# zhouxian/act3d-chained-diffuser

Measured on AMD Instinct MI355X. Metric: train samples/sec (Act3D keypose fwd+bwd+AdamW step), higher is better.
Workload: dtype fp16 / bf16 MFMA on two-part operands (x = hi + lo; fp32 accumulate) in attention; fp32-accurate linears (f32 MFMA; bf16x3 MFMA from 4096 rows); bf16 frozen backbone + FPN; 1 GPU; Act3D keypose training step, 18-PerAct-task shapes: 4 cameras 256x256, 3 ghost-point levels, 1000 ghost points (333/level), E=60, frozen synthetic CLIP-RN50-shaped backbone + trainable FPN included in the step; per_gpu_batch_keyframes=64, global_batch=64, parallelism=dp1, hipgraph=True, backbone_prefetch=True

## Files before the change

act3d-chained-diffuser_amd/csrc/conv3x3.hip:

```cpp
#include "a3d_common.h"
#include "../../include/act3d_hip.h"

namespace a3d {

constexpr int C3_TH = 8, C3_TW = 32;
constexpr int C3_HW = C3_TW + 2, C3_HP = (C3_TH + 2) * C3_HW;
constexpr int C3_XL = (C3_HP * 4 + 255) / 256;

__device__ __forceinline__ int c3_woff(int row, int seg) { return row * 32 + ((seg ^ (((row >> 1) & 1) | (((row >> 4) & 1) << 1))) << 3); }
__device__ __forceinline__ int c3_xoff(int hp, int hx, int seg) { return hp * 32 + ((seg ^ ((hx >> 1) & 3)) << 3); }

typedef float c3_f32x2 __attribute__((ext_vector_type(2)));
typedef short c3_s16x2 __attribute__((ext_vector_type(2)));
typedef unsigned int c3_u32x4 __attribute__((ext_vector_type(4)));

struct C3Cursor {
  int img, ty, tx;
  __device__ __forceinline__ void advance(int dimg, int dty, int dtx, int tiles_y, int tiles_x) {
    tx += dtx;
    if (tx >= tiles_x) { tx -= tiles_x; ++ty; }
    ty += dty;
    if (ty >= tiles_y) { ty -= tiles_y; ++img; }
    img += dimg;
  }
};

constexpr int c3_lds_bytes(int halves, int nt) { return halves * 9 * 16 * nt * 64 + 2 * C3_HP * 64 + 2 * 32 * halves * 4; }

template <int HALVES, int NT, int D, bool LIST = false>
__global__ __launch_bounds__(256, (2 * c3_lds_bytes(HALVES, NT) <= 160 * 1024 ? 2 : 1)) void conv3x3_stream_kernel(
    const unsigned short* __restrict__ x, const unsigned short* __restrict__ w, const float* __restrict__ in_scale,
    const float* __restrict__ in_shift, int in_relu, unsigned short* __restrict__ y, float* __restrict__ partial, int nimg, int H,
    int W, int ctot, const int* __restrict__ tlist = nullptr) {
  constexpr int CIN = 32 * HALVES, COUT = 16 * NT;
  const int co0 = blockIdx.y * COUT;
  static_assert(D % HALVES == 0, "the half of a step must be a compile-time function of its slot");
  extern __shared__ __attribute__((aligned(16))) unsigned short smem_c3[];
  unsigned short* Ws = smem_c3;
  unsigned short* Xs = Ws + HALVES * 9 * COUT * 32;
  float* scS = reinterpret_cast<float*>(Xs + 2 * C3_HP * 32);
  const int t = threadIdx.x, lane = t & 63, wave = t >> 6;
  const int li = lane & 15, g = lane >> 4;
  const int nwg = gridDim.x;
  const int lb = (nwg & 7) == 0 ? (int)(blockIdx.x & 7) * (nwg >> 3) + (int)(blockIdx.x >> 3) : (int)blockIdx.x;
  const int tiles_x = W / C3_TW, tiles_y = H / C3_TH, tpi = tiles_x * tiles_y;
  const int ntiles = LIST ? __builtin_amdgcn_readfirstlane(tlist[-2]) : nimg * tpi;
  for (int i = t; i < HALVES * 9 * COUT * 4; i += 256) {
    const int seg = i & 3, r = i >> 2, co = r % COUT, tap = (r / COUT) % 9, h = r / (COUT * 9);
    *reinterpret_cast<uint4*>(&Ws[c3_woff((h * 9 + tap) * COUT + co, seg)]) =
        *reinterpret_cast<const uint4*>(w + ((size_t)(co0 + co) * 9 + tap) * CIN + h * 32 + seg * 8);
  }
  for (int i = t; i < CIN; i += 256) { scS[i] = in_scale ? in_scale[i] : 1.f; scS[CIN + i] = in_scale ? in_shift[i] : 0.f; }
  const int seg_t = t & 3;
  int hy[C3_XL], hx[C3_XL];
#pragma unroll
  for (int i = 0; i < C3_XL; ++i) {
    const int hp = (t + i * 256) >> 2;
    hy[i] = hp / C3_HW;
    hx[i] = hp - hy[i] * C3_HW;
  }
  c3_f32x2 ssum[NT][2], ssq[NT][2];
#pragma unroll
  for (int a = 0; a < NT; ++a)
#pragma unroll
    for (int r = 0; r < 2; ++r) { ssum[a][r] = c3_f32x2{0.f, 0.f}; ssq[a][r] = c3_f32x2{0.f, 0.f}; }
  const int my_tiles = lb < ntiles ? (ntiles - lb + nwg - 1) / nwg : 0;
  const int total = my_tiles * HALVES;
  const int dimg = nwg / tpi, dty = (nwg - dimg * tpi) / tiles_x, dtx = nwg - dimg * tpi - dty * tiles_x;
  C3Cursor cl;
  auto from_list = [&](int ordinal) {
    const int e = __builtin_amdgcn_readfirstlane(tlist[lb + ordinal * nwg]);
    return C3Cursor{e >> 16, (e >> 8) & 255, e & 255};
  };
  if (LIST) {
    cl = my_tiles > 0 ? from_list(0) : C3Cursor{0, 0, 0};
  } else {
    cl.img = lb / tpi;
    cl.ty = (lb - cl.img * tpi) / tiles_x;
    cl.tx = lb - cl.img * tpi - cl.ty * tiles_x;
  }
  C3Cursor cc = cl;
  int lk = 0, lhalf = 0;
  int ck = 0;
  auto load_next = [&](uint4 (&r)[C3_XL]) {
    const int y0 = cl.ty * C3_TH, x0 = cl.tx * C3_TW;
    const char* base = reinterpret_cast<const char*>(x + (size_t)cl.img * H * W * CIN + lhalf * 32);
#pragma unroll
    for (int i = 0; i < C3_XL; ++i) {
      const int iy = min(max(y0 - 1 + hy[i], 0), H - 1), ix = min(max(x0 - 1 + hx[i], 0), W - 1);
      const unsigned int off = (unsigned int)((iy * W + ix) * CIN + seg_t * 8) * 2u;
      r[i] = *reinterpret_cast<const uint4*>(base + off);
    }
    if (++lhalf == HALVES) {
      lhalf = 0;
      if (lk + 1 < my_tiles) {
        ++lk;
        if (LIST) cl = from_list(lk); else cl.advance(dimg, dty, dtx, tiles_y, tiles_x);
      }
    }
  };
  const c3_s16x2 relu_lo = in_relu ? c3_s16x2{0, 0} : c3_s16x2{(short)-32768, (short)-32768};
  auto stage = [&](int buf, int half, const uint4 (&r)[C3_XL]) {
    const int y0 = cc.ty * C3_TH, x0 = cc.tx * C3_TW;
    const int k0 = half * 32 + seg_t * 8;
    c3_f32x2 sc[4], sh[4];
#pragma unroll
    for (int j = 0; j < 4; ++j) {
      sc[j] = c3_f32x2{scS[k0 + 2 * j], scS[k0 + 2 * j + 1]};
      sh[j] = c3_f32x2{scS[CIN + k0 + 2 * j], scS[CIN + k0 + 2 * j + 1]};
    }
#pragma unroll
    for (int i = 0; i < C3_XL; ++i) {
      const int hp = (t + i * 256) >> 2;
      const int iy = y0 - 1 + hy[i], ix = x0 - 1 + hx[i];
      const bool inside = (unsigned)iy < (unsigned)H && (unsigned)ix < (unsigned)W;
      unsigned int u[4] = {r[i].x, r[i].y, r[i].z, r[i].w};
#pragma unroll
      for (int j = 0; j < 4; ++j) {
        c3_f32x2 v = {__uint_as_float(u[j] << 16), __uint_as_float(u[j] & 0xFFFF0000u)};
        v = v * sc[j] + sh[j];
        const c3_s16x2 pk = __builtin_elementwise_max(__builtin_bit_cast(c3_s16x2, pk_bf16(v.x, v.y)), relu_lo);
        u[j] = inside ? __builtin_bit_cast(unsigned int, pk) : 0u;
      }
      if (hp < C3_HP) *reinterpret_cast<c3_u32x4*>(&Xs[buf * C3_HP * 32 + c3_xoff(hp, hx[i], seg_t)]) = c3_u32x4{u[0], u[1], u[2], u[3]};
    }
  };
  int xo[4][3], woff[NT];
#pragma unroll
  for (int tm = 0; tm < 4; ++tm)
#pragma unroll
    for (int kw = 0; kw < 3; ++kw) {
      const int col = (tm & 1) * 16 + li + kw;
      xo[tm][kw] = c3_xoff((2 * wave + (tm >> 1)) * C3_HW + col, col, g);
    }
#pragma unroll
  for (int tn = 0; tn < NT; ++tn) woff[tn] = c3_woff((li >> 2) * (4 * NT) + tn * 4 + (li & 3), g);
  if (total > 0) {
    uint4 xr[D][C3_XL];
#pragma unroll
    for (int j = 0; j < D; ++j) load_next(xr[j]);
    f32x4 acc[NT][4];
#pragma unroll
    for (int a = 0; a < NT; ++a)
#pragma unroll
      for (int b = 0; b < 4; ++b) acc[a][b] = f32x4{0.f, 0.f, 0.f, 0.f};
    __syncthreads();
    for (int s0 = 0; s0 < total; s0 += D) {
#pragma unroll
      for (int j = 0; j < D; ++j) {
        const int s = s0 + j;
        if (s >= total) break;
        const int half = j % HALVES, buf = s & 1;
        stage(buf, half, xr[j]);
        load_next(xr[j]);
        __syncthreads();
        const unsigned short* Xb = Xs + buf * C3_HP * 32;
        const unsigned short* Wb = Ws + half * 9 * COUT * 32;
        auto taps_of_row = [&](int kh) {
#pragma unroll
          for (int kw = 0; kw < 3; ++kw) {
            s16x8 xa[4], wb[NT];
#pragma unroll
            for (int tm = 0; tm < 4; ++tm) xa[tm] = *reinterpret_cast<const s16x8*>(&Xb[xo[tm][kw] + kh * (C3_HW * 32)]);
#pragma unroll
            for (int tn = 0; tn < NT; ++tn) wb[tn] = *reinterpret_cast<const s16x8*>(&Wb[(kh * 3 + kw) * COUT * 32 + woff[tn]]);
#pragma unroll
            for (int tn = 0; tn < NT; ++tn)
#pragma unroll
              for (int tm = 0; tm < 4; ++tm) acc[tn][tm] = mfma_bf16_16x16x32(wb[tn], xa[tm], acc[tn][tm]);
          }
        };
#pragma unroll
        for (int kh = 0; kh < 3; ++kh) taps_of_row(kh);
        if (half == HALVES - 1) {
          const int y0 = cc.ty * C3_TH, x0 = cc.tx * C3_TW;
#pragma unroll
          for (int tm = 0; tm < 4; ++tm) {
            const int oy = y0 + 2 * wave + (tm >> 1), ox = x0 + (tm & 1) * 16 + li;
            unsigned int pk[2 * NT];
#pragma unroll
            for (int tn = 0; tn < NT; ++tn) {
#pragma unroll
              for (int r2 = 0; r2 < 2; ++r2) {
                const unsigned int u = pk_bf16(acc[tn][tm][2 * r2], acc[tn][tm][2 * r2 + 1]);
                const c3_f32x2 v = {__uint_as_float(u << 16), __uint_as_float(u & 0xFFFF0000u)};
                ssum[tn][r2] += v;
                ssq[tn][r2] += v * v;
                pk[2 * tn + r2] = u;
              }
              acc[tn][tm] = f32x4{0.f, 0.f, 0.f, 0.f};
            }
            char* ybase = reinterpret_cast<char*>(y + (size_t)cc.img * H * W * ctot + co0);
            c3_u32x4* dst = reinterpret_cast<c3_u32x4*>(ybase + (unsigned int)((oy * W + ox) * ctot + g * (4 * NT)) * 2u);
#pragma unroll
            for (int q = 0; q < NT / 2; ++q) dst[q] = c3_u32x4{pk[4 * q], pk[4 * q + 1], pk[4 * q + 2], pk[4 * q + 3]};
          }
          if (LIST) { if (++ck < my_tiles) cc = from_list(ck); } else cc.advance(dimg, dty, dtx, tiles_y, tiles_x);
        }
      }
    }
  }
  if (LIST) {
    const int nzero = __builtin_amdgcn_readfirstlane(tlist[-1]);
    const int last = nimg * tpi - 1;
    for (int k = lb; k < nzero; k += nwg) {
      const int e = __builtin_amdgcn_readfirstlane(tlist[last - k]);
      const int img = e >> 16, oy = ((e >> 8) & 255) * C3_TH + (t >> 5), ox = (e & 255) * C3_TW + (t & 31);
      char* ybase = reinterpret_cast<char*>(y + (size_t)img * H * W * ctot + co0);
      c3_u32x4* dst = reinterpret_cast<c3_u32x4*>(ybase + (unsigned int)((oy * W + ox) * ctot) * 2u);
#pragma unroll
      for (int q = 0; q < COUT / 8; ++q) dst[q] = c3_u32x4{0u, 0u, 0u, 0u};
    }
  }
  if (!partial) return;
  __syncthreads();
  float* redS = reinterpret_cast<float*>(Xs);
  float* redQ = redS + 4 * COUT;
#pragma unroll
  for (int tn = 0; tn < NT; ++tn)
#pragma unroll
    for (int r = 0; r < 4; ++r) {
      float sv = ssum[tn][r >> 1][r & 1], q = ssq[tn][r >> 1][r & 1];
#pragma unroll
      for (int o = 1; o < 16; o <<= 1) { sv += __shfl_xor(sv, o, 64); q += __shfl_xor(q, o, 64); }
      if (li == 0) { redS[wave * COUT + g * (4 * NT) + tn * 4 + r] = sv; redQ[wave * COUT + g * (4 * NT) + tn * 4 + r] = q; }
    }
  __syncthreads();
  if (t < COUT) {
    float sv = 0.f, q = 0.f;
#pragma unroll
    for (int j = 0; j < 4; ++j) { sv += redS[j * COUT + t]; q += redQ[j * COUT + t]; }
    float* p = partial + (size_t)blockIdx.x * 2 * ctot + co0;
    p[t] = sv;
    p[ctot + t] = q;
  }
}

__global__ __launch_bounds__(256) void c3_mark_tiles_kernel(const long long* __restrict__ idx, long long ntok, int k, int ncam, int H,
                                                          int W, unsigned char* __restrict__ mask) {
  const long long i = (long long)blockIdx.x * 256 + threadIdx.x;
  if (i >= ntok) return;
  const long long p = idx[i];
  const int b = (int)(i / k);
  const int cam = (int)(p / ((long long)H * W));
  const int rem = (int)(p - (long long)cam * H * W);
  const int h = rem / W, w0 = rem - h * W;
  const int tiles_x = W / C3_TW, tiles_y = H / C3_TH;
  const int img = b * ncam + cam;
  const int ty0 = max(h - 1, 0) / C3_TH, ty1 = min(h + 1, H - 1) / C3_TH, tx0 = max(w0 - 1, 0) / C3_TW, tx1 = min(w0 + 1, W - 1) / C3_TW;
  for (int ty = ty0; ty <= ty1; ++ty)
    for (int tx = tx0; tx <= tx1; ++tx) mask[((size_t)img * tiles_y + ty) * tiles_x + tx] = 1;
}

__global__ __launch_bounds__(1024) void c3_compact_tiles_kernel(const unsigned char* __restrict__ mask, int ntiles, int tiles_x,
                                                              int tiles_y, int* __restrict__ tlist) {
  __shared__ int wsum[16];
  __shared__ int carry;
  const int t = threadIdx.x, lane = t & 63, wave = t >> 6;
  const int tpi = tiles_x * tiles_y;
  if (t == 0) carry = 0;
  __syncthreads();
  for (int base = 0; base < ntiles; base += 1024) {
    const int id = base + t;
    const int on = (id < ntiles && mask[id]) ? 1 : 0;
    const unsigned long long bal = __ballot(on);
    const int before = __popcll(bal & ((1ull << lane) - 1ull));
    if (lane == 0) wsum[wave] = __popcll(bal);
    __syncthreads();
    int off = carry;
    for (int w2 = 0; w2 < wave; ++w2) off += wsum[w2];
    if (id < ntiles) {
      const int img = id / tpi, r = id - img * tpi, ty = r / tiles_x, tx = r - ty * tiles_x;
      const int e = (img << 16) | (ty << 8) | tx;
      const int pos_on = off + before;
      if (on) tlist[pos_on] = e; else tlist[ntiles - 1 - (id - pos_on)] = e;
    }
    __syncthreads();
    if (t == 0) { int tot = 0; for (int w2 = 0; w2 < 16; ++w2) tot += wsum[w2]; carry += tot; }
    __syncthreads();
  }
  if (t == 0) { tlist[-2] = carry; tlist[-1] = ntiles - carry; }
}

}

using namespace a3d;

static int c3_cblock(int Cin, int Cout) {
  static const bool split = !(getenv("A3D_C3_SPLIT") && atoi(getenv("A3D_C3_SPLIT")) == 0);
  return (Cin == 64 && Cout == 64 && split) ? 32 : Cout;
}
static size_t c3_lds(int Cin, int Cout) { return (size_t)c3_lds_bytes(Cin / 32, c3_cblock(Cin, Cout) / 16); }
static bool c3_serves(int Cin, int Cout, int H, int W) {
  const bool ch = (Cin == 32 && (Cout == 32 || Cout == 64)) || (Cin == 64 && Cout == 64);
  return ch && H > 0 && W > 0 && (H % C3_TH) == 0 && (W % C3_TW) == 0;
}
static int c3_slabs(size_t nimg, int H, int W, int Cin, int Cout) {
  const size_t ntiles = nimg * (size_t)(H / C3_TH) * (size_t)(W / C3_TW);
  const int per_cu = 2 * c3_lds(Cin, Cout) <= 160 * 1024 ? 2 : 1;
  const int yblocks = Cout / c3_cblock(Cin, Cout);
  return (int)std::min<size_t>(ntiles, (size_t)std::max(8, 256 * per_cu / yblocks));
}

extern "C" int a3d_conv3x3_serves(int Cin, int Cout, int H, int W) { return c3_serves(Cin, Cout, H, W) ? 1 : 0; }

extern "C" int a3d_conv3x3_nslab(size_t nimg, int H, int W, int Cin, int Cout) {
  if (nimg == 0 || !c3_serves(Cin, Cout, H, W)) return 0;
  return c3_slabs(nimg, H, W, Cin, Cout);
}

extern "C" int a3d_conv3x3_bn_fwd(const void* x, const void* w, const float* in_scale, const float* in_shift, int in_relu, void* y,
                                  float* partial, size_t nimg, int H, int W, int Cin, int Cout, void* stream) {
  if (!x || !w || !y || nimg == 0 || nimg * (size_t)(H > 0 ? H : 1) * (size_t)(W > 0 ? W : 1) / 256 >= (size_t)(1 << 30) || (size_t)(H > 0 ? H : 1) * (size_t)(W > 0 ? W : 1) * 128 >= ((size_t)1 << 31) || !c3_serves(Cin, Cout, H, W) || (in_scale && !in_shift) ||
      ((((uintptr_t)x | (uintptr_t)w | (uintptr_t)y) & 15) != 0)) {
    set_error("a3d_conv3x3_bn_fwd: bad argument (images=%zu H=%d W=%d Cin=%d Cout=%d; served: 32 -> 32, 32 -> 64, 64 -> 64 channels, "
              "H a multiple of 8, W a multiple of 32 -- a3d_conv3x3_serves; 16-byte aligned operands)", nimg, H, W, Cin, Cout);
    return A3D_ERR_ARG;
  }
  hipStream_t s = (hipStream_t)stream;
  const unsigned short* xs = (const unsigned short*)x;
  const unsigned short* ws = (const unsigned short*)w;
  unsigned short* ys = (unsigned short*)y;
  const int slabs = c3_slabs(nimg, H, W, Cin, Cout);
  const size_t lds = c3_lds(Cin, Cout);
#define A3D_C3S(HV, NTV, DV)                                                                                                        \
  do {                                                                                                                           \
    static bool once = false;                                                                                                    \
    if (!once) { (void)hipFuncSetAttribute((const void*)conv3x3_stream_kernel<HV, NTV, DV>, hipFuncAttributeMaxDynamicSharedMemorySize, 128 * 1024); once = true; } \
    hipLaunchKernelGGL((conv3x3_stream_kernel<HV, NTV, DV>), dim3(slabs, Cout / c3_cblock(Cin, Cout)), dim3(256), lds, s, xs, ws, in_scale, in_shift, in_relu, ys, partial, (int)nimg, H, W, Cout); \
  } while (0)
  if (Cin == 32 && Cout == 32) A3D_C3S(1, 2, 3);
  else if (Cin == 32 && Cout == 64) A3D_C3S(1, 4, 2);
  else if (c3_cblock(Cin, Cout) == 32) A3D_C3S(2, 2, 2);
  else A3D_C3S(2, 4, 2);
#undef A3D_C3S
  return check_launch("a3d_conv3x3_bn_fwd");
}

extern "C" size_t a3d_conv3x3_tile_count(size_t nimg, int H, int W) {
  return (H > 0 && W > 0 && (H % C3_TH) == 0 && (W % C3_TW) == 0) ? nimg * (size_t)(H / C3_TH) * (size_t)(W / C3_TW) : 0;
}
extern "C" size_t a3d_conv3x3_dgrad_tiles_ws_ints(size_t nimg, int H, int W) { return a3d_conv3x3_tile_count(nimg, H, W) + 4; }

extern "C" int a3d_conv3x3_mark_tiles(const long long* idx, int B, int k, int ncam, int H, int W, unsigned char* mask, void* stream) {
  if (!idx || !mask || B <= 0 || k <= 0 || ncam <= 0 || a3d_conv3x3_tile_count(1, H, W) == 0 || H / C3_TH > 255 || W / C3_TW > 255) {
    set_error("a3d_conv3x3_mark_tiles: bad argument (B=%d k=%d ncam=%d H=%d W=%d; H a multiple of 8, W of 32)", B, k, ncam, H, W);
    return A3D_ERR_ARG;
  }
  const long long ntok = (long long)B * k;
  hipLaunchKernelGGL(c3_mark_tiles_kernel, dim3((unsigned)((ntok + 255) / 256)), dim3(256), 0, (hipStream_t)stream, idx, ntok, k, ncam, H, W, mask);
  return check_launch("a3d_conv3x3_mark_tiles");
}

extern "C" int a3d_conv3x3_dgrad_tiles(const void* dy, const void* wt, const unsigned char* mask, int* ws, void* dx, size_t nimg, int H,
                                       int W, void* stream) {
  if (!dy || !wt || !mask || !ws || !dx || nimg == 0 || nimg >= 32768 || !c3_serves(64, 64, H, W) || H / C3_TH > 255 || W / C3_TW > 255 ||
      (size_t)H * (size_t)W * 128 >= ((size_t)1 << 31) || ((((uintptr_t)dy | (uintptr_t)wt | (uintptr_t)dx) & 15) != 0)) {
    set_error("a3d_conv3x3_dgrad_tiles: bad argument (images=%zu H=%d W=%d; 64 channels, H a multiple of 8, W of 32, < 32768 images)", nimg, H, W);
    return A3D_ERR_ARG;
  }
  hipStream_t s = (hipStream_t)stream;
  const int ntiles = (int)a3d_conv3x3_tile_count(nimg, H, W);
  int* tlist = ws + 2;
  hipLaunchKernelGGL(c3_compact_tiles_kernel, dim3(1), dim3(1024), 0, s, mask, ntiles, W / C3_TW, H / C3_TH, tlist);
  int rc = check_launch("a3d_conv3x3_dgrad_tiles(compact)");
  if (rc) return rc;
  const int slabs = c3_slabs(nimg, H, W, 64, 64);
  const size_t lds = c3_lds(64, 64);
  const int cb = c3_cblock(64, 64);
  static bool once = false;
  if (cb == 32) {
    if (!once) { (void)hipFuncSetAttribute((const void*)conv3x3_stream_kernel<2, 2, 2, true>, hipFuncAttributeMaxDynamicSharedMemorySize, 128 * 1024); once = true; }
    hipLaunchKernelGGL((conv3x3_stream_kernel<2, 2, 2, true>), dim3(slabs, 2), dim3(256), lds, s, (const unsigned short*)dy, (const unsigned short*)wt,
                       (const float*)nullptr, (const float*)nullptr, 0, (unsigned short*)dx, (float*)nullptr, (int)nimg, H, W, 64, (const int*)tlist);
  } else {
    if (!once) { (void)hipFuncSetAttribute((const void*)conv3x3_stream_kernel<2, 4, 2, true>, hipFuncAttributeMaxDynamicSharedMemorySize, 128 * 1024); once = true; }
    hipLaunchKernelGGL((conv3x3_stream_kernel<2, 4, 2, true>), dim3(slabs, 1), dim3(256), lds, s, (const unsigned short*)dy, (const unsigned short*)wt,
                       (const float*)nullptr, (const float*)nullptr, 0, (unsigned short*)dx, (float*)nullptr, (int)nimg, H, W, 64, (const int*)tlist);
  }
  return check_launch("a3d_conv3x3_dgrad_tiles");
}
```

include/act3d_hip.h:

```cpp
#ifndef ACT3D_HIP_H
#define ACT3D_HIP_H
#include <stddef.h>
#include <stdint.h>
#ifdef __cplusplus
extern "C" {
#endif

int a3d_version(void);
const char* a3d_last_error_string(void);

int a3d_linear_fwd(const float* X, int ldx, const float* W, int ldw, const float* bias, float* Y, int ldy,
                   const float* mask, int ldm, int M, int N, int K, int act, int w_transposed, void* stream);
int a3d_linear_wgrad(const float* dY, int lddy, const float* X, int ldx, float* dW, int lddw, float* db, int M,
                     int N, int K, void* stream);
size_t a3d_linear_wgrad_ws_bytes(int M, int N, int K, int has_bias);
int a3d_linear_wgrad_ws(const float* dY, int lddy, const float* X, int ldx, float* dW, int lddw, float* db, int M,
                        int N, int K, float* ws, size_t ws_bytes, void* stream);
int a3d_add_layernorm_fwd(const float* A, const float* R, const float* gamma, const float* beta, float* Y,
                          float* mean, float* rstd, int M, int E, float eps, void* stream);
int a3d_add_layernorm_bwd(const float* A, const float* R, const float* gamma, const float* mean, const float* rstd,
                          const float* dY, float* dS, float* dgamma, float* dbeta, int M, int E, void* stream);

int a3d_linear_wgrad_partials(const float* dY, int lddy, const float* X, int ldx, int has_bias, int M, int N, int K,
                              float* ws, size_t ws_bytes, int* nsplit_out, void* stream);
int a3d_add_layernorm_bwd_partials_count(int M, int E);
int a3d_add_layernorm_bwd_partials(const float* A, const float* R, const float* gamma, const float* mean, const float* rstd,
                                   const float* dY, float* dS, float* partials, int M, int E, void* stream);
int a3d_colsum_rows_partials(const float* src, int B, int S, int k, int ld, int C, float* ws, void* stream);
typedef struct {
  const float* partial;
  float* dst;
  float* bias;
  int nsplit, slab_stride, count, row_len, dst_stride, group_len;
} A3dGradReduceRec;
int a3d_grad_reduce_table_plan(const A3dGradReduceRec* host_table, int nrec, int* nwg_out);
int a3d_grad_reduce_table_upload(A3dGradReduceRec* dev_table, const A3dGradReduceRec* host_table, int nrec, void* stream);
int a3d_grad_reduce_table(const A3dGradReduceRec* dev_table, int nrec, int nwg, void* stream);

int a3d_rope_split_qk(const float* Y, int ldy, const float* xyz, const float* freq, float scale, void* dst, int B,
                      int N, int Npad, int E, int H, void* stream);
int a3d_split_vt(const float* Y, int ldy, void* dst, int B, int N, int Npad, int E, int H, void* stream);
int a3d_rope_split(const float* Y, int ldy, const float* xyz, const float* freq, float scale, void* rows_out,
                   int rows_width, void* planes_out, int B, int N, int Npad, int E, int H, void* stream);
int a3d_proj_rope_split(const float* X, int ldx, const float* W, int ldw, const float* bias, int K, const float* xyz0,
                        float scale0, void* rows0, int rows0_width, void* planes0, const float* xyz1, float scale1,
                        void* rows1, int rows1_width, void* planes1, const float* freq, int B, int N, int Npad, int E,
                        int H, void* stream);
int a3d_rope_merge_bwd(const float* dR, int nsplit, const float* xyz, const float* freq, float scale, float* dY,
                       int ldy, int B, int N, int Npad, int E, int H, void* stream);

int a3d_attn_fwd(const void* Qs, const void* Ks, const void* Vt, const unsigned char* kmask, float* O, float* LSE,
                 float* ws, int B, int H, int Lq, int Lqp, int S, int Sp, int nsplit, void* stream);
size_t a3d_attn_fwd_ws_floats(int B, int H, int Lqp, int nsplit);
int a3d_attn_bwd_bf16(const void* Qs, const void* Qt, const void* Ks, const void* Kt, const void* Vs,
                      const unsigned char* kmask, const float* O, const float* dO, const float* LSE, void* dOs,
                      void* dOt, float* D, float* dQp, float* dK, float* dV, int B, int H, int Lq, int Lqp, int S,
                      int Sp, int nsplit, void* stream);

int a3d_dropout(const float* x, float* y, size_t n, const unsigned long long* drop_state, unsigned int site, float p,
                void* stream);
int a3d_linear_fwd_drop(const float* X, int ldx, const float* W, int ldw, const float* bias, float* Y, int ldy,
                        const float* mask, int ldm, int M, int N, int K, int act, int w_transposed,
                        const unsigned long long* drop_state, unsigned int site, float p, void* stream);
int a3d_add_layernorm_bwd_drop(const float* A, const float* R, const float* gamma, const float* mean, const float* rstd,
                               const float* dY, float* dS, float* dS_drop, float* dgamma, float* dbeta, int M, int E,
                               const unsigned long long* drop_state, unsigned int site, float p, void* stream);
int a3d_dropout_mask(unsigned char* out, size_t n, const unsigned long long* drop_state, unsigned int c2, unsigned int c1,
                     unsigned int site, float p, void* stream);
int a3d_rope_split16(const float* Y, int ldy, const float* xyz, const float* freq, float scale, void* rows_out,
                     void* planes_out, int plane_parts, int B, int N, int Npad, int E, int H, void* stream);
int a3d_proj_rope_split16(const float* X, int ldx, const float* W, int ldw, const float* bias, int K, const float* xyz0,
                          float scale0, void* rows0, void* planes0, int parts0, const float* xyz1, float scale1, void* rows1,
                          void* planes1, int parts1, const float* freq, int B, int N, int Npad, int E, int H, void* stream);
int a3d_ctx_kv_proj16_splits(int B, int Npad);
int a3d_ctx_kv_proj16(const float* X, int ldx, const float* xyz, const float* W0, const float* bias0, void* Krows0, void* Vrows0,
                      const float* W1, const float* bias1, void* Krows1, void* Vrows1, int ldw, const float* freq, int nl, int B,
                      int N, int Npad, int E, int H, int nsplit, void* stream);
int a3d_attn16_fwd(const void* Qr, const void* Kr, const void* Vp, const unsigned char* kmask, float* O, float* LSE2,
                   float* ws, int B, int H, int Lq, int Lqp, int S, int Sp, int nsplit,
                   const unsigned long long* drop_state, unsigned int drop_site, float drop_p, void* stream);
int a3d_attn16_fwd_rows(const void* Qr, const void* Kr, const void* Vr, const unsigned char* kmask, float* O, float* LSE2,
                        float* ws, int B, int H, int Lq, int Lqp, int S, int Sp, int nsplit,
                        const unsigned long long* drop_state, unsigned int drop_site, float drop_p, int nograd, void* stream);
size_t a3d_attn16_bwd_pack_bytes(int B, int H, int Lqp);
int a3d_attn16_bwd(const void* Qr, const void* Qp, const void* Kr, const void* Kp, const void* Vr,
                   const unsigned char* kmask, const float* O, const float* dO, const float* LSE2, void* dOr, void* pack,
                   float* D, int* rexp, float* dQp, float* dK, float* dV, int B, int H, int Lq, int Lqp, int S, int Sp,
                   int nsplit, const unsigned long long* drop_state, unsigned int drop_site, float drop_p, void* stream);

size_t a3d_attn8_operand_bytes(int B, int H, int Sp);
int a3d_attn8_fwd(const void* Qr, const void* Kr, const void* Vp, void* ops8, const unsigned char* kmask, float* O,
                  float* LSE2, float* ws, int B, int H, int Lq, int Lqp, int S, int Sp, int nsplit, void* stream);

int a3d_attn_fwd_dropout(const void* Qs, const void* Ks, const void* Vt, const unsigned char* kmask, float* O, float* LSE,
                         float* ws, int B, int H, int Lq, int Lqp, int S, int Sp, int nsplit,
                         const unsigned long long* drop_state, unsigned int site, float p, void* stream);
int a3d_attn_bwd_bf16_dropout(const void* Qs, const void* Qt, const void* Ks, const void* Kt, const void* Vs,
                              const unsigned char* kmask, const float* O, const float* dO, const float* LSE, void* dOs,
                              void* dOt, float* D, float* dQp, float* dK, float* dV, int B, int H, int Lq, int Lqp, int S,
                              int Sp, int nsplit, const unsigned long long* drop_state, unsigned int site, float p,
                              void* stream);

size_t a3d_sq_fwd_ws_floats(int B, int H, int E, int nsplit);
int a3d_sq_attn_fwd(const float* X, const float* xyz, const float* Wk, int ldw, const float* bk, const float* Wv, int ldwv,
                    const float* bv, const float* qrot, const float* freq, float* ws, float* xbar, float* lse, float* o, int B,
                    int S, int E, int H, int nsplit, void* stream);
size_t a3d_sq_bwd_ws_floats(int B, int H, int E, int nsplit);
int a3d_sq_attn_bwd(const float* X, const float* xyz, const float* Wk, int ldw, const float* bk, const float* Wv, int ldwv,
                    const float* qrot, const float* freq, const float* xbar, const float* lse, const float* dO, float* ws,
                    float* dX, float* dqp, float* dWk, int lddwk, float* dbk, float* dWv, int lddwv, float* dbv, int B, int S,
                    int E, int H, int nsplit, void* stream);
int a3d_sq_attn_bwd_acc(const float* X, const float* xyz, const float* Wk, int ldw, const float* bk, const float* Wv, int ldwv,
                        const float* qrot, const float* freq, const float* xbar, const float* lse, const float* dO, float* ws,
                        float* dX, float* dqp, float* dWk, int lddwk, float* dbk, float* dWv, int lddwv, float* dbv, int B, int S,
                        int E, int H, int nsplit, int accumulate_dX, void* stream);
int a3d_sq_wgrad_reduce(const float* partial, int nsplit, float* dW, int lddw, float* db, int E, void* stream);

int a3d_pcd_downsample(const float* pcd, float* out_xyz, int B, int C, int Hin, int Win, int factor, void* stream);
size_t a3d_knn_topk_ws_bytes(int B, int N);
int a3d_knn_topk(const float* pos, const float* xyz, void* ws, long long* idx_out, float* dist_out, int B, int N,
                 int k, void* stream);
int a3d_traj_nn_topk(const float* traj_xyz, int L, const float* xyz, void* ws, long long* idx_out, float* dist_out, int B,
                     int N, int k, void* stream);
int a3d_build_context(const float* feat, const long long* idx, const float* extra, float* ctx, int B, int Npts,
                      int k, int X, int W, void* stream);
int a3d_build_context_bwd(const float* dctx, const long long* idx, float* dfeat, float* dextra, int B, int Npts,
                          int k, int X, int W, int accumulate, void* stream);

int a3d_build_context_bf16(const void* feat, int ldf, const long long* idx, const float* extra, const float* bias, float* ctx,
                           int B, int Npts, int k, int X, int W, void* stream);
int a3d_build_context_bwd_bf16(const float* dctx, const long long* idx, void* dfeat, int ldf, float* dextra, int B,
                               int Npts, int k, int X, int W, int accumulate, void* stream);
size_t a3d_conv3x3_wgrad_tokens_ws_floats(void);
int a3d_conv3x3_wgrad_tokens(const void* X, const long long* idx, const float* G, int g_rows, int E, float* ws, float* dW,
                             int accumulate, int B, int k, int ncam, int H, int W, void* stream);
size_t a3d_conv3x3_tile_count(size_t images, int H, int W);
size_t a3d_conv3x3_dgrad_tiles_ws_ints(size_t images, int H, int W);
int a3d_conv3x3_mark_tiles(const long long* idx, int B, int k, int ncam, int H, int W, unsigned char* mask, void* stream);
int a3d_conv3x3_dgrad_tiles(const void* dy, const void* wt, const unsigned char* mask, int* ws, void* dx, size_t images, int H, int W,
                            void* stream);
size_t a3d_colsum_rows_ws_floats(int B, int k, int C);
int a3d_colsum_rows(const float* src, int B, int S, int k, int ld, int C, float* out, int nout, float* ws, void* stream);

int a3d_mask_logits_fwd(const float* q, const float* F, float* out, int B, int Ng, int E, void* stream);
int a3d_mask_logits_bwd(const float* q, const float* F, const float* dlog, float* dF, float* dq, int B, int Ng,
                        int E, int accumulate_dF, void* stream);
int a3d_argmax_gather(const float* logits, const float* ghost, long long* top_idx, float* pos, int B, int Ng,
                      void* stream);
int a3d_soft_ce_loss(const float* ghost, const float* gt, const float* logits, float* loss_b, float* loss,
                     float* dlogits, int B, int Ng, float spread, float label_smoothing, float coeff, void* stream);
int a3d_elem_loss(const float* pred, const float* target, int n, int kind, float coeff, float* loss, float* grad,
                  void* stream);
int a3d_scale_by_scalar(const float* x, const float* scalar, float* y, size_t n, void* stream);
int a3d_quat_sigmoid_fwd(const float* pred, float* rot, float* grip, int B, void* stream);
int a3d_quat_sigmoid_bwd(const float* pred, const float* drot, const float* dgrip, float* dpred, int B, void* stream);
int a3d_ortho6d_sigmoid_fwd(const float* pred, float* rot, float* grip, int B, void* stream);
int a3d_ortho6d_sigmoid_bwd(const float* pred, const float* drot, const float* dgrip, float* dpred, int B, void* stream);
int a3d_select_row_fwd(const float* x, const long long* idx, float* y, int B, int N, int W, void* stream);
int a3d_select_row_bwd(const float* dy, const long long* idx, float* dx, int B, int N, int W, void* stream);
int a3d_sample_ghost_points(const unsigned long long* state, const float* bounds, const float* anchor, float radius,
                            float* out, int B, int Ng, int level, int max_attempts, void* stream);
int a3d_rng_advance(unsigned long long* state, unsigned long long n, void* stream);
void a3d_philox4x32_10_host(const uint32_t* ctr, const uint32_t* key, uint32_t* out);
void a3d_sincos_host(const float* x, float* sn, float* cs, size_t n);
int a3d_adamw_step(float* p, const float* g, float* m, float* v, float* step, const long long* seg_off, float* seg_state,
                   int nseg, size_t n, size_t n_nodecay, float lr, float beta1, float beta2, float eps, float wd_nodecay,
                   float wd_decay, float grad_scale, void* stream);
int a3d_adamw_ema_step(float* p, const float* g, float* m, float* v, float* ema, float* step, const long long* seg_off,
                       float* seg_state, float* ema_state, int nseg, size_t n, size_t n_nodecay, float lr, float beta1, float beta2,
                       float eps, float wd_nodecay, float wd_decay, float grad_scale, float ema_decay, float ema_warmup,
                       void* stream);
#define A3D_ADAMW_CLIP_WS_DOUBLES 256
int a3d_adamw_clip_step(float* p, const float* g, float* m, float* v, float* ema, float* step, const long long* seg_off,
                        float* seg_state, float* ema_state, float* clip_state, double* clip_ws, int nseg, size_t n, size_t n_nodecay,
                        float lr, float beta1, float beta2, float eps, float wd_nodecay, float wd_decay, float grad_scale,
                        float ema_decay, float ema_warmup, float max_norm, void* stream);
#define A3D_LR_CONSTANT 0
#define A3D_LR_LINEAR 1
#define A3D_LR_COSINE 2
int a3d_adamw_sched_step(float* p, const float* g, float* m, float* v, float* ema, float* step, const long long* seg_off,
                         float* seg_state, float* ema_state, float* clip_state, double* clip_ws, float* lr_state, int nseg, size_t n,
                         size_t n_nodecay, int decay_kind, double warmup_steps, double total_steps, double min_ratio, float beta1,
                         float beta2, float eps, float wd_nodecay, float wd_decay, float grad_scale, float ema_decay, float ema_warmup,
                         float max_norm, void* stream);
int a3d_swap_f32(float* a, float* b, size_t n, void* stream);

typedef struct {
  const float *wv, *bv;
  const float *wo, *bo;
  const float *g1, *b1;
  const float *w1, *c1, *w2, *c2;
  const float *g2, *b2;
} a3d_qs_params;
typedef struct {
  float *dwv, *dbv, *dwo, *dbo, *dg1, *db1, *dw1, *dc1, *dw2, *dc2, *dg2, *db2;
} a3d_qs_grads;
int a3d_qs_pre_fwd(const float* x, const float* wq, const float* bq, const float* xyz, const float* freq, float scale, float* qrot,
                   int B, int E, int H, void* stream);
int a3d_qs_pre_bwd(const float* dqp, int nsplit, const float* xyz, const float* freq, float scale, const float* x, const float* wq,
                   float* dwq, float* dbq, float* dx, int B, int E, int H, void* stream);
size_t a3d_qs_save_floats(int B, int E);
int a3d_qs_post_fwd(const float* xbar, const float* resid, const a3d_qs_params* p, float* save, float* y, int B, int E, int H,
                    void* stream);
int a3d_qs_post_bwd(const float* dy, const float* resid, const float* xbar, const float* save, const a3d_qs_params* p,
                    const a3d_qs_grads* gr, float* dxbar, float* cD, float* dresid, int B, int E, int H, void* stream);

int a3d_ddpm_add_noise(const float* x0, const float* noise, const long long* t, const float* acp_pos,
                       const float* acp_rot, float* out, int B, int L, int D, int npos, void* stream);
int a3d_ddpm_step(const float* model_out, const float* sample, const float* noise, const float* cond_data,
                  const unsigned char* cond_mask, const float* coef_pos, const float* coef_rot, float* out, int rows,
                  int D, int npos, int t, void* stream);
int a3d_ddpm_step_sched(const float* model_out, const float* sample, const float* noise, const float* cond_data,
                        const unsigned char* cond_mask, const float* coef_pos, const float* coef_rot, float* out, int rows,
                        int D, int npos, int row, int terminal, void* stream);
int a3d_ddpm_step_hist(const float* model_out, const float* sample, const float* noise, const float* cond_data,
                       const unsigned char* cond_mask, const float* coef_pos, const float* coef_rot, float* out, int rows,
                       int D, int npos, int row, int terminal, float* hist, const float* kappa_pos, const float* kappa_rot,
                       void* stream);
int a3d_adaln_fwd(const float* x, const float* mod, float* y, int B, int L, int E, void* stream);
int a3d_adaln_bwd(const float* x, const float* mod, const float* dy, float* dx, float* dmod, int B, int L, int E,
                  void* stream);
int a3d_sinusoidal_emb(const float* x, float* out, int n, int E, void* stream);
int a3d_silu_fwd(const float* x, float* y, size_t n, void* stream);
int a3d_silu_bwd(const float* x, const float* dy, float* dx, size_t n, void* stream);
int a3d_add_rows(const float* x, const float* r, float* y, int B, int L, int E, void* stream);
int a3d_add_rows_bwd(const float* dy, float* dr, int B, int L, int E, void* stream);
int a3d_traj_update(const float* traj, const float* upd, float* out, int rows, int D, int npos, void* stream);

int a3d_pose_to_signal(const float* pose, const float* bounds, float* out, int n, int extra, void* stream);
int a3d_signal_to_pose(const float* signal, const float* bounds, float* out, int n, int extra, void* stream);
int a3d_traj_condition(const float* curr, int ldc, const float* goal, int ldg, const float* bounds, const unsigned char* tmask,
                       const float* init_noise, float* cg, float* gg, float* cond_data, unsigned char* cond_mask,
                       unsigned char* kmask, float* traj, int B, int G, int L, int Dp, int use_goal, void* stream);
#define A3D_TRAJ_PINS_MAX 32
int a3d_traj_pins(const float* poses, int ldp, const int* index, const unsigned char* channels, const float* bounds,
                  const unsigned char* tmask, const float* init_noise, float* cond_data, unsigned char* cond_mask, float* traj,
                  unsigned char* applied, int B, int G, int P, int L, int Dp, int use_goal, void* stream);
int a3d_traj_rank(const float* poses, const unsigned char* tmask, const float* goal, int ldg, const float* bounds,
                  float w_consensus, float w_goal, float w_smooth, float w_length, float w_bounds, float rot_weight, int* best,
                  int* order, float* scores, float* terms, float* selected, int B, int G, int L, int Dp, void* stream);
int a3d_traj_rank_extra(const float* poses, const unsigned char* tmask, const float* goal, int ldg, const float* bounds,
                        float w_consensus, float w_goal, float w_smooth, float w_length, float w_bounds, float rot_weight, int* best,
                        int* order, float* scores, float* terms, float* selected, int B, int G, int L, int Dp, const float* extra,
                        float w_extra, void* stream);
size_t a3d_traj_clearance_ws_floats(int B, int G, int L, int n_points, int n_chunks);
int a3d_traj_clearance(const float* poses, const unsigned char* tmask, const float* scene, const unsigned char* scene_mask, int n_cam,
                       int n_pix, float margin, int skip_head, int skip_tail, float* nearest, float* clearance, float* ws,
                       int n_chunks, int B, int G, int L, int Dp, void* stream);
size_t a3d_traj_guide_ws_floats(int B, int G, int L, int n_points, int n_chunks);
int a3d_traj_guide(float* traj, int D, const unsigned char* tmask, const unsigned char* cond_mask, const float* bounds,
                   const float* scene, const unsigned char* scene_mask, int n_cam, int n_pix, float margin, int skip_head,
                   int skip_tail, float push, float smooth, float* nearest, float* ws, int n_chunks, int B, int G, int L,
                   void* stream);
int a3d_traj_errors(const float* pred, const float* gt, float* cols, int B, int L, int D, void* stream);
int a3d_keypose_errors(const float* pos, const float* rot, const float* grip, const float* gt, int ldgt, float* cols, int B,
                       int nlev, int symmetric, void* stream);
int a3d_sym_quat_loss(const float* q, const float* gt, int ldgt, float coeff, float* loss, float* grad, int B, void* stream);

typedef struct {
  const float *enc_w0, *enc_b0, *enc_w1, *enc_b1;
  const float* sem;
  const float* lang_kv;
  int S_lang;
  const float *q_w, *q_b, *out_w, *out_b, *ln_g, *ln_b;
} a3d_dn_head_params;
typedef struct {
  const float* sem;
  const float* mod;
  const float *q_w, *q_b;
  const float* freq;
  const void* Kf;
  const unsigned short* Vt;
} a3d_dn_cross_params;
typedef struct {
  const float *c_out_w, *c_out_b, *c_ln_g, *c_ln_b;
  const float* sem;
  const float *s_mod, *s_in_w, *s_in_b, *s_out_w, *s_out_b, *s_ln_g, *s_ln_b;
  const float* freq;
  const unsigned char* kmask;
  const float *f_mod, *f_w1, *f_b1, *f_w2, *f_b2, *f_ln_g, *f_ln_b;
  int F;
} a3d_dn_rest_params;
typedef struct {
  const float *pos_w0, *pos_b0, *pos_w1, *pos_b1, *rot_w0, *rot_b0, *rot_w1, *rot_b1;
  const float *noise, *cond_data;
  const unsigned char* cond_mask;
  const float *coef_pos, *coef_rot;
  float* hist;
  const float *kappa_pos, *kappa_rot;
} a3d_dn_tail_params;
int a3d_dn_head(const float* traj, int D, const a3d_dn_head_params* p, float* x_out, int B, int L, int E, int H, void* stream);
size_t a3d_dn_cross_ws_floats(int B, int H, int nsplit);
int a3d_dn_cross(const float* x, const float* traj, int D, const a3d_dn_cross_params* p, float* ws, int B, int L, int E,
                 int H, int S, int Sp, int nsplit, void* stream);
int a3d_dn_rest(const float* x_in, const float* traj, int D, const float* ws, const a3d_dn_rest_params* p, float* x_out,
                int B, int L, int E, int H, int nsplit, void* stream);
int a3d_dn_tail(const float* pos_feats, const float* rot_feats, const float* traj, int D, const a3d_dn_tail_params* p,
                float* traj_out, int B, int L, int E, int t_step, void* stream);
int a3d_dn_tail_sched(const float* pos_feats, const float* rot_feats, const float* traj, int D, const a3d_dn_tail_params* p,
                      float* traj_out, int B, int L, int E, int row, int terminal, void* stream);
typedef struct {
  a3d_dn_cross_params cross;
  a3d_dn_rest_params rest;
} a3d_dn_layer_params;
int a3d_dn_persist_splits(int H, int nsplit);
size_t a3d_dn_persist_kvx_floats(int B, int L, int E);
size_t a3d_dn_persist_xbuf_floats(int B, int L);
int a3d_dn_persist_prof(const int* sync, int B, int L, int n_layers, int nsteps, long long* out256);
size_t a3d_dn_persist_sync_ints(int B, int L, int n_layers, int nsteps);
int a3d_dn_persist(const a3d_dn_layer_params* layers_dev, int n_traj, int n_pos, int n_rot, const a3d_dn_head_params* head,
                   const a3d_dn_tail_params* tail, float* traj, float* qbuf, float* part, float* kvx, float* xbuf, int* sync, int B,
                   int L, int D, int E, int H, int S, int Sp, int nsplit, int t_first, int nsteps, void* stream);
int a3d_dn_persist_sched(const a3d_dn_layer_params* layers_dev, int n_traj, int n_pos, int n_rot, const a3d_dn_head_params* head,
                         const a3d_dn_tail_params* tail, float* traj, float* qbuf, float* part, float* kvx, float* xbuf, int* sync,
                         int B, int L, int D, int E, int H, int S, int Sp, int nsplit, int row_first, int nsteps, int n_rows,
                         int last_terminal, void* stream);
int a3d_dn_persist_group_of(int B, int L, int n_cand, int traj, int* out5);
int a3d_dn_persist_group(const a3d_dn_layer_params* layers_dev, int n_traj, int n_pos, int n_rot, const a3d_dn_head_params* head,
                         const a3d_dn_tail_params* tail, float* traj, float* qbuf, float* part, float* kvx, float* xbuf, int* sync,
                         int B, int L, int D, int E, int H, int S, int Sp, int nsplit, int row_first, int nsteps, int n_rows,
                         int last_terminal, int n_cand, void* stream);
int a3d_dbg_dn_prof(long long* out18);
int a3d_rope_rows_f32(const float* Y, int ldy, const float* xyz, const float* freq, float scale, float* out, int B, int N,
                      int Npad, int E, int H, void* stream);

int a3d_bn_nslab(size_t rows, int C);
int a3d_bn_stats(const void* x, float* partial , size_t rows, int C, int nslab, void* stream);
int a3d_bn_finalize(const float* partial, int nslab, size_t rows, int C, float eps, float momentum, const float* gamma,
                    const float* beta, float* running_mean, float* running_var, float* scale, float* shift, int train,
                    void* stream);
int a3d_bn_apply(const void* x, const void* residual, const float* res_scale, const float* res_shift, const float* scale,
                 const float* shift, void* y, size_t rows, int C, int relu, void* stream);
int a3d_bn_apply_pool2(const void* x, const void* residual, const float* scale, const float* shift, void* y_full,
                       void* y_pool, int N, int H, int W, int C, int relu, void* stream);
int a3d_bn_grid_cap(int cap);
int a3d_upsample2_add_fwd(const void* lat, const void* top, const float* bias, int nbias, void* y, int N, int H, int W, int C,
                          void* stream);
size_t a3d_upsample2_add_bwd_ws_floats(int N, int H, int W, int C);
int a3d_upsample2_add_bwd(const void* dy, void* dtop, float* dbias, int nbias, float* ws, int N, int H, int W, int C,
                          void* stream);

int a3d_rgb_normalize_nhwc_bf16(const float* x, const float* mean, const float* stdv, void* y, size_t N, int H, int W,
                                void* stream);

int a3d_dbg_mfma_bf16(const void* A16x32, const void* B32x16, float* D16x16, void* stream);
int a3d_dbg_mfma_f32(const float* A16x4, const float* B4x16, float* D16x16, void* stream);
int a3d_dbg_cvt_pk_bf16(const float* in, void* out, int npairs, void* stream);

int a3d_conv1x1_streams(int K, int N);
int a3d_conv1x1_nslab(size_t M, int K, int N);
int a3d_conv1x1_bn_fwd(const void* x, const void* w, const float* in_scale, const float* in_shift, int in_relu, void* y,
                       float* partial, size_t M, int K, int N, void* stream);
int a3d_conv1x1_topdown_serves(int K, int N);
int a3d_conv1x1_topdown_fwd(const void* x, const void* w, const float* bias, int nbias, const void* top, void* y, size_t images,
                            int H, int W, int K, int N, void* stream);
int a3d_conv1x1_bn_residual_serves(int K, int N);
int a3d_conv1x1_bn_residual_fwd(const void* x, const void* w, const float* in_scale, const float* in_shift, int in_relu,
                                const float* out_scale, const float* out_shift, const void* res, const float* res_scale,
                                const float* res_shift, int relu, int round_conv, void* y, size_t M, int K, int N, void* stream);
int a3d_bn_gram_nslab(size_t M, int K);
int a3d_bn_gram(const void* x, const float* in_scale, const float* in_shift, int in_relu, float* gpart, float* spart, size_t M, int K,
                int nslab, void* stream);
int a3d_bn_gram_stats(const float* gpart, const float* spart, int nslab, const void* w, int K, int N, double* work, float* stats,
                      void* stream);
int a3d_conv1x1_deep_mode(int mode);
int a3d_stem_conv_nslab(size_t images, int H, int W);
int a3d_stem_conv_bn_fwd(const float* rgb, const float* mean, const float* stdv, const void* w, void* y, float* partial, size_t images,
                         int H, int W, void* stream);

int a3d_conv3x3_serves(int Cin, int Cout, int H, int W);
int a3d_conv3x3_nslab(size_t images, int H, int W, int Cin, int Cout);
int a3d_conv3x3_bn_fwd(const void* x, const void* w, const float* in_scale, const float* in_shift, int in_relu, void* y,
                       float* partial, size_t images, int H, int W, int Cin, int Cout, void* stream);

int a3d_resize_crop(const float* src, float* dst, const int* params, int frames, int planes, int H, int W, float scale,
                    float shift, void* stream);

#ifdef __cplusplus
}
#endif
#endif
```

Before: 3695 samples/s.

## Pair two tile streams per 512-thread workgroup sharing conv3x3 weights; skip identity BN staging

For the 64->64 3x3 conv (forward and dgrad), each workgroup now runs two 256-thread groups that share one LDS copy of the full 64-output weight block while processing alternating tiles with separate input buffers. This replaces the previous split into two 32-channel y-blocks or a single 64-channel group, cutting redundant weight loads and LDS use per tile. A new IDENT path skips the scale/shift/relu conversion when no input affine is applied and copies raw bf16 into LDS. The risks are lower occupancy from the larger workgroup, idle groups at the tail, and barriers shared across both groups. Both paths are on by default and can be turned off with an environment variable.

Result: no change. 3716 samples/s, median of 5 (+0.6%).

```diff
diff --git a/act3d-chained-diffuser_amd/csrc/conv3x3.hip b/act3d-chained-diffuser_amd/csrc/conv3x3.hip
--- a/act3d-chained-diffuser_amd/csrc/conv3x3.hip
+++ b/act3d-chained-diffuser_amd/csrc/conv3x3.hip
@@ -25,32 +25,37 @@
   }
 };
 
-constexpr int c3_lds_bytes(int halves, int nt) { return halves * 9 * 16 * nt * 64 + 2 * C3_HP * 64 + 2 * 32 * halves * 4; }
-
-template <int HALVES, int NT, int D, bool LIST = false>
-__global__ __launch_bounds__(256, (2 * c3_lds_bytes(HALVES, NT) <= 160 * 1024 ? 2 : 1)) void conv3x3_stream_kernel(
+constexpr int c3_lds_bytes(int halves, int nt, int groups = 1) { return halves * 9 * 16 * nt * 64 + groups * 2 * C3_HP * 64 + 2 * 32 * halves * 4; }
+
+template <int HALVES, int NT, int D, bool LIST = false, bool PAIR = false, bool IDENT = false>
+__global__ __launch_bounds__(PAIR ? 512 : 256, (!PAIR && 2 * c3_lds_bytes(HALVES, NT) <= 160 * 1024 ? 2 : 1)) void conv3x3_stream_kernel(
     const unsigned short* __restrict__ x, const unsigned short* __restrict__ w, const float* __restrict__ in_scale,
     const float* __restrict__ in_shift, int in_relu, unsigned short* __restrict__ y, float* __restrict__ partial, int nimg, int H,
     int W, int ctot, const int* __restrict__ tlist = nullptr) {
   constexpr int CIN = 32 * HALVES, COUT = 16 * NT;
+  constexpr int NTHR = PAIR ? 512 : 256, NGRP = PAIR ? 2 : 1;
+  static_assert(!PAIR || (HALVES == 2 && NT == 4), "the paired instance is the 64 -> 64 one");
   const int co0 = blockIdx.y * COUT;
   static_assert(D % HALVES == 0, "the half of a step must be a compile-time function of its slot");
   extern __shared__ __attribute__((aligned(16))) unsigned short smem_c3[];
   unsigned short* Ws = smem_c3;
-  unsigned short* Xs = Ws + HALVES * 9 * COUT * 32;
-  float* scS = reinterpret_cast<float*>(Xs + 2 * C3_HP * 32);
-  const int t = threadIdx.x, lane = t & 63, wave = t >> 6;
+  unsigned short* Xs0 = Ws + HALVES * 9 * COUT * 32;
+  float* scS = reinterpret_cast<float*>(Xs0 + NGRP * 2 * C3_HP * 32);
+  const int t8 = threadIdx.x, grp = PAIR ? __builtin_amdgcn_readfirstlane(t8 >> 8) : 0;
+  const int t = t8 & 255, lane = t & 63, wave = t >> 6;
+  unsigned short* Xs = Xs0 + grp * (2 * C3_HP * 32);
   const int li = lane & 15, g = lane >> 4;
   const int nwg = gridDim.x;
   const int lb = (nwg & 7) == 0 ? (int)(blockIdx.x & 7) * (nwg >> 3) + (int)(blockIdx.x >> 3) : (int)blockIdx.x;
   const int tiles_x = W / C3_TW, tiles_y = H / C3_TH, tpi = tiles_x * tiles_y;
   const int ntiles = LIST ? __builtin_amdgcn_readfirstlane(tlist[-2]) : nimg * tpi;
-  for (int i = t; i < HALVES * 9 * COUT * 4; i += 256) {
+  for (int i = t8; i < HALVES * 9 * COUT * 4; i += NTHR) {
     const int seg = i & 3, r = i >> 2, co = r % COUT, tap = (r / COUT) % 9, h = r / (COUT * 9);
     *reinterpret_cast<uint4*>(&Ws[c3_woff((h * 9 + tap) * COUT + co, seg)]) =
         *reinterpret_cast<const uint4*>(w + ((size_t)(co0 + co) * 9 + tap) * CIN + h * 32 + seg * 8);
   }
-  for (int i = t; i < CIN; i += 256) { scS[i] = in_scale ? in_scale[i] : 1.f; scS[CIN + i] = in_scale ? in_shift[i] : 0.f; }
+  if (!IDENT)
+    for (int i = t8; i < CIN; i += NTHR) { scS[i] = in_scale ? in_scale[i] : 1.f; scS[CIN + i] = in_scale ? in_shift[i] : 0.f; }
   const int seg_t = t & 3;
   int hy[C3_XL], hx[C3_XL];
 #pragma unroll
@@ -64,20 +69,23 @@
   for (int a = 0; a < NT; ++a)
 #pragma unroll
     for (int r = 0; r < 2; ++r) { ssum[a][r] = c3_f32x2{0.f, 0.f}; ssq[a][r] = c3_f32x2{0.f, 0.f}; }
-  const int my_tiles = lb < ntiles ? (ntiles - lb + nwg - 1) / nwg : 0;
-  const int total = my_tiles * HALVES;
-  const int dimg = nwg / tpi, dty = (nwg - dimg * tpi) / tiles_x, dtx = nwg - dimg * tpi - dty * tiles_x;
+  const int wg_tiles = lb < ntiles ? (ntiles - lb + nwg - 1) / nwg : 0;
+  const int my_tiles = PAIR ? (wg_tiles + 1 - grp) >> 1 : wg_tiles;
+  const int total = ((wg_tiles + NGRP - 1) / NGRP) * HALVES;
+  const int adv = nwg * NGRP;
+  const int dimg = adv / tpi, dty = (adv - dimg * tpi) / tiles_x, dtx = adv - dimg * tpi - dty * tiles_x;
   C3Cursor cl;
   auto from_list = [&](int ordinal) {
-    const int e = __builtin_amdgcn_readfirstlane(tlist[lb + ordinal * nwg]);
+    const int e = __builtin_amdgcn_readfirstlane(tlist[lb + (ordinal * NGRP + grp) * nwg]);
     return C3Cursor{e >> 16, (e >> 8) & 255, e & 255};
   };
   if (LIST) {
     cl = my_tiles > 0 ? from_list(0) : C3Cursor{0, 0, 0};
   } else {
-    cl.img = lb / tpi;
-    cl.ty = (lb - cl.img * tpi) / tiles_x;
-    cl.tx = lb - cl.img * tpi - cl.ty * tiles_x;
+    const int first = my_tiles > 0 ? lb + grp * nwg : lb;
+    cl.img = first / tpi;
+    cl.ty = (first - cl.img * tpi) / tiles_x;
+    cl.tx = first - cl.img * tpi - cl.ty * tiles_x;
   }
   C3Cursor cc = cl;
   int lk = 0, lhalf = 0;
@@ -102,6 +110,17 @@
   const c3_s16x2 relu_lo = in_relu ? c3_s16x2{0, 0} : c3_s16x2{(short)-32768, (short)-32768};
   auto stage = [&](int buf, int half, const uint4 (&r)[C3_XL]) {
     const int y0 = cc.ty * C3_TH, x0 = cc.tx * C3_TW;
+    if constexpr (IDENT) {
+#pragma unroll
+      for (int i = 0; i < C3_XL; ++i) {
+        const int hp = (t + i * 256) >> 2;
+        const int iy = y0 - 1 + hy[i], ix = x0 - 1 + hx[i];
+        const bool inside = (unsigned)iy < (unsigned)H && (unsigned)ix < (unsigned)W;
+        const c3_u32x4 v = inside ? c3_u32x4{r[i].x, r[i].y, r[i].z, r[i].w} : c3_u32x4{0u, 0u, 0u, 0u};
+        if (hp < C3_HP) *reinterpret_cast<c3_u32x4*>(&Xs[buf * C3_HP * 32 + c3_xoff(hp, hx[i], seg_t)]) = v;
+      }
+      return;
+    }
     const int k0 = half * 32 + seg_t * 8;
     c3_f32x2 sc[4], sh[4];
 #pragma unroll
@@ -151,9 +170,11 @@
         const int s = s0 + j;
         if (s >= total) break;
         const int half = j % HALVES, buf = s & 1;
-        stage(buf, half, xr[j]);
+        const bool active = !PAIR || ck < my_tiles;
+        if (active) stage(buf, half, xr[j]);
         load_next(xr[j]);
         __syncthreads();
+        if (!active) continue;
         const unsigned short* Xb = Xs + buf * C3_HP * 32;
         const unsigned short* Wb = Ws + half * 9 * COUT * 32;
         auto taps_of_row = [&](int kh) {
@@ -195,7 +216,8 @@
 #pragma unroll
             for (int q = 0; q < NT / 2; ++q) dst[q] = c3_u32x4{pk[4 * q], pk[4 * q + 1], pk[4 * q + 2], pk[4 * q + 3]};
           }
-          if (LIST) { if (++ck < my_tiles) cc = from_list(ck); } else cc.advance(dimg, dty, dtx, tiles_y, tiles_x);
+          ++ck;
+          if (LIST) { if (ck < my_tiles) cc = from_list(ck); } else cc.advance(dimg, dty, dtx, tiles_y, tiles_x);
         }
       }
     }
@@ -203,7 +225,7 @@
   if (LIST) {
     const int nzero = __builtin_amdgcn_readfirstlane(tlist[-1]);
     const int last = nimg * tpi - 1;
-    for (int k = lb; k < nzero; k += nwg) {
+    for (int k = lb + grp * nwg; k < nzero; k += adv) {
       const int e = __builtin_amdgcn_readfirstlane(tlist[last - k]);
       const int img = e >> 16, oy = ((e >> 8) & 255) * C3_TH + (t >> 5), ox = (e & 255) * C3_TW + (t & 31);
       char* ybase = reinterpret_cast<char*>(y + (size_t)img * H * W * ctot + co0);
@@ -214,8 +236,10 @@
   }
   if (!partial) return;
   __syncthreads();
-  float* redS = reinterpret_cast<float*>(Xs);
-  float* redQ = redS + 4 * COUT;
+  constexpr int NW = 4 * NGRP;
+  const int wv = t8 >> 6;
+  float* redS = reinterpret_cast<float*>(Xs0);
+  float* redQ = redS + NW * COUT;
 #pragma unroll
   for (int tn = 0; tn < NT; ++tn)
 #pragma unroll
@@ -223,16 +247,16 @@
       float sv = ssum[tn][r >> 1][r & 1], q = ssq[tn][r >> 1][r & 1];
 #pragma unroll
       for (int o = 1; o < 16; o <<= 1) { sv += __shfl_xor(sv, o, 64); q += __shfl_xor(q, o, 64); }
-      if (li == 0) { redS[wave * COUT + g * (4 * NT) + tn * 4 + r] = sv; redQ[wave * COUT + g * (4 * NT) + tn * 4 + r] = q; }
+      if (li == 0) { redS[wv * COUT + g * (4 * NT) + tn * 4 + r] = sv; redQ[wv * COUT + g * (4 * NT) + tn * 4 + r] = q; }
     }
   __syncthreads();
-  if (t < COUT) {
+  if (t8 < COUT) {
     float sv = 0.f, q = 0.f;
 #pragma unroll
-    for (int j = 0; j < 4; ++j) { sv += redS[j * COUT + t]; q += redQ[j * COUT + t]; }
+    for (int j = 0; j < NW; ++j) { sv += redS[j * COUT + t8]; q += redQ[j * COUT + t8]; }
     float* p = partial + (size_t)blockIdx.x * 2 * ctot + co0;
-    p[t] = sv;
-    p[ctot + t] = q;
+    p[t8] = sv;
+    p[ctot + t8] = q;
   }
 }
 
@@ -290,7 +314,24 @@
   static const bool split = !(getenv("A3D_C3_SPLIT") && atoi(getenv("A3D_C3_SPLIT")) == 0);
   return (Cin == 64 && Cout == 64 && split) ? 32 : Cout;
 }
+static int c3_mode = getenv("A3D_C3_PAIR") ? (atoi(getenv("A3D_C3_PAIR")) != 0 ? 1 : 0) : 1;
+extern "C" int a3d_conv3x3_mode(int mode) {
+  const int prev = c3_mode;
+  if (mode >= 0) c3_mode = mode > 0 ? 1 : 0;
+  return prev;
+}
 static size_t c3_lds(int Cin, int Cout) { return (size_t)c3_lds_bytes(Cin / 32, c3_cblock(Cin, Cout) / 16); }
+constexpr int C3_PAIR_LDS = c3_lds_bytes(2, 4, 2);
+static_assert(C3_PAIR_LDS <= 160 * 1024, "one workgroup may declare 163,840 B of LDS");
+template <int HV, int NTV, int DV, bool LIST, bool PAIR, bool IDENT>
+static void c3_launch(int slabs, int yblocks, hipStream_t s, const unsigned short* x, const unsigned short* w, const float* in_scale,
+                      const float* in_shift, int in_relu, unsigned short* y, float* partial, int nimg, int H, int W, int ctot, const int* tlist) {
+  constexpr int lds = c3_lds_bytes(HV, NTV, PAIR ? 2 : 1);
+  static bool once = false;
+  if (!once) { (void)hipFuncSetAttribute((const void*)conv3x3_stream_kernel<HV, NTV, DV, LIST, PAIR, IDENT>, hipFuncAttributeMaxDynamicSharedMemorySize, PAIR ? lds : 128 * 1024); once = true; }
+  hipLaunchKernelGGL((conv3x3_stream_kernel<HV, NTV, DV, LIST, PAIR, IDENT>), dim3(slabs, yblocks), dim3(PAIR ? 512 : 256), lds, s, x, w, in_scale, in_shift,
+                     in_relu, y, partial, nimg, H, W, ctot, tlist);
+}
 static bool c3_serves(int Cin, int Cout, int H, int W) {
   const bool ch = (Cin == 32 && (Cout == 32 || Cout == 64)) || (Cin == 64 && Cout == 64);
   return ch && H > 0 && W > 0 && (H % C3_TH) == 0 && (W % C3_TW) == 0;
@@ -322,17 +363,16 @@
   const unsigned short* ws = (const unsigned short*)w;
   unsigned short* ys = (unsigned short*)y;
   const int slabs = c3_slabs(nimg, H, W, Cin, Cout);
-  const size_t lds = c3_lds(Cin, Cout);
-#define A3D_C3S(HV, NTV, DV)                                                                                                        \
-  do {                                                                                                                           \
-    static bool once = false;                                                                                                    \
-    if (!once) { (void)hipFuncSetAttribute((const void*)conv3x3_stream_kernel<HV, NTV, DV>, hipFuncAttributeMaxDynamicSharedMemorySize, 128 * 1024); once = true; } \
-    hipLaunchKernelGGL((conv3x3_stream_kernel<HV, NTV, DV>), dim3(slabs, Cout / c3_cblock(Cin, Cout)), dim3(256), lds, s, xs, ws, in_scale, in_shift, in_relu, ys, partial, (int)nimg, H, W, Cout); \
-  } while (0)
-  if (Cin == 32 && Cout == 32) A3D_C3S(1, 2, 3);
-  else if (Cin == 32 && Cout == 64) A3D_C3S(1, 4, 2);
-  else if (c3_cblock(Cin, Cout) == 32) A3D_C3S(2, 2, 2);
-  else A3D_C3S(2, 4, 2);
+  const bool pair = c3_mode != 0 && Cin == 64;
+  const bool ident = c3_mode != 0 && !in_scale && !in_relu;
+  const int yblocks = pair ? 1 : Cout / c3_cblock(Cin, Cout);
+#define A3D_C3S(HV, NTV, DV, PAIRV, IDENTV) \
+  c3_launch<HV, NTV, DV, false, PAIRV, IDENTV>(slabs, yblocks, s, xs, ws, in_scale, in_shift, in_relu, ys, partial, (int)nimg, H, W, Cout, nullptr)
+  if (Cin == 32 && Cout == 32) { if (ident) A3D_C3S(1, 2, 3, false, true); else A3D_C3S(1, 2, 3, false, false); }
+  else if (Cin == 32 && Cout == 64) { if (ident) A3D_C3S(1, 4, 2, false, true); else A3D_C3S(1, 4, 2, false, false); }
+  else if (pair) { if (ident) A3D_C3S(2, 4, 2, true, true); else A3D_C3S(2, 4, 2, true, false); }
+  else if (c3_cblock(Cin, Cout) == 32) A3D_C3S(2, 2, 2, false, false);
+  else A3D_C3S(2, 4, 2, false, false);
 #undef A3D_C3S
   return check_launch("a3d_conv3x3_bn_fwd");
 }
@@ -366,17 +406,11 @@
   int rc = check_launch("a3d_conv3x3_dgrad_tiles(compact)");
   if (rc) return rc;
   const int slabs = c3_slabs(nimg, H, W, 64, 64);
-  const size_t lds = c3_lds(64, 64);
-  const int cb = c3_cblock(64, 64);
-  static bool once = false;
-  if (cb == 32) {
-    if (!once) { (void)hipFuncSetAttribute((const void*)conv3x3_stream_kernel<2, 2, 2, true>, hipFuncAttributeMaxDynamicSharedMemorySize, 128 * 1024); once = true; }
-    hipLaunchKernelGGL((conv3x3_stream_kernel<2, 2, 2, true>), dim3(slabs, 2), dim3(256), lds, s, (const unsigned short*)dy, (const unsigned short*)wt,
-                       (const float*)nullptr, (const float*)nullptr, 0, (unsigned short*)dx, (float*)nullptr, (int)nimg, H, W, 64, (const int*)tlist);
-  } else {
-    if (!once) { (void)hipFuncSetAttribute((const void*)conv3x3_stream_kernel<2, 4, 2, true>, hipFuncAttributeMaxDynamicSharedMemorySize, 128 * 1024); once = true; }
-    hipLaunchKernelGGL((conv3x3_stream_kernel<2, 4, 2, true>), dim3(slabs, 1), dim3(256), lds, s, (const unsigned short*)dy, (const unsigned short*)wt,
-                       (const float*)nullptr, (const float*)nullptr, 0, (unsigned short*)dx, (float*)nullptr, (int)nimg, H, W, 64, (const int*)tlist);
-  }
+#define A3D_C3L(NTV, PAIRV, IDENTV, YB) \
+  c3_launch<2, NTV, 2, true, PAIRV, IDENTV>(slabs, YB, s, (const unsigned short*)dy, (const unsigned short*)wt, nullptr, nullptr, 0, (unsigned short*)dx, nullptr, (int)nimg, H, W, 64, tlist)
+  if (c3_mode != 0) A3D_C3L(4, true, true, 1);
+  else if (c3_cblock(64, 64) == 32) A3D_C3L(2, false, false, 2);
+  else A3D_C3L(4, false, false, 1);
+#undef A3D_C3L
   return check_launch("a3d_conv3x3_dgrad_tiles");
 }
diff --git a/include/act3d_hip.h b/include/act3d_hip.h
--- a/include/act3d_hip.h
+++ b/include/act3d_hip.h
@@ -372,6 +372,7 @@
 int a3d_conv3x3_nslab(size_t images, int H, int W, int Cin, int Cout);
 int a3d_conv3x3_bn_fwd(const void* x, const void* w, const float* in_scale, const float* in_shift, int in_relu, void* y,
                        float* partial, size_t images, int H, int W, int Cin, int Cout, void* stream);
+int a3d_conv3x3_mode(int mode);
 
 int a3d_resize_crop(const float* src, float* dst, const int* params, int frames, int planes, int H, int W, float scale,
                     float shift, void* stream);
```
